# maniacs-ops/ringpop-go

Measured on AMD Instinct MI355X. Metric: simulated member-rounds/sec at 64k members, higher is better.
Workload: dtype u32; 1 GPU; config3_cascade: 65536 members, 655 killed at r=10; rounds 5-592 timed (steady state, kill, suspect wave; faulty wave from r>=35 in window); members=65536, live_member_rounds=38153303, parallelism=1 GPU

## Files before the change

include/swimsim.h:

```cpp
#ifndef SWIMSIM_H
#define SWIMSIM_H
#include <stddef.h>
#include <stdint.h>

#ifdef __cplusplus
extern "C" {
#endif

#define SWIMSIM_ABI_VERSION 13

enum {
    SWIMSIM_OK = 0,
    SWIMSIM_EINVAL = -1,
    SWIMSIM_ENOMEM = -2,
    SWIMSIM_EHIP = -3,
    SWIMSIM_ECAPACITY = -4,
    SWIMSIM_ERANGE = -5
};

enum { SWIMSIM_ALIVE = 0, SWIMSIM_SUSPECT = 1, SWIMSIM_FAULTY = 2, SWIMSIM_LEAVE = 3, SWIMSIM_TOMBSTONE = 4,
       SWIMSIM_UNKNOWN = 7 };
#define SWIMSIM_SOURCE_NONE (-1)

typedef struct swimsim_config {
// ... 14 lines not shown
    uint64_t message_pool_bytes;
    uint32_t observer_begin, observer_end;
    const struct swimsim_tuning *tuning;
} swimsim_config;

typedef struct swimsim_tuning {
    int32_t hot_slots;
    int32_t dense_slots;
    int32_t cs_async;
    int32_t cs_async_rows;
    int32_t cs_narrow_rows;
    int32_t cs_ref;
    int32_t fault_inject;
    int32_t defer_test;
    int32_t cs_defer;
} swimsim_tuning;

enum {
    SWIMSIM_EV_KILL = 1,
    SWIMSIM_EV_REVIVE = 2,
    SWIMSIM_EV_REINCARNATE = 3,
    SWIMSIM_EV_LEAVE = 4,
    SWIMSIM_EV_PARTITION = 5,
    SWIMSIM_EV_HEAL = 6,
    SWIMSIM_EV_REAP = 7,
    SWIMSIM_EV_CLOCK = 8
};
typedef struct swimsim_event { uint32_t round; uint32_t kind; int32_t a; int32_t b; } swimsim_event;

enum {
// ... 127 lines not shown
```

ringpop-go_amd/csrc/swimsim_device.h:

```cpp
#pragma once
#include <hip/hip_runtime.h>
#include <stdint.h>

namespace swimdev {

constexpr uint32_t ST_ALIVE = 0, ST_SUSPECT = 1, ST_FAULTY = 2, ST_LEAVE = 3, ST_TOMB = 4, ST_UNKNOWN = 7;
constexpr uint32_t SRC_NONE = 0xFFFFFFFFu;
constexpr uint32_t NO_DEADLINE = 0xFFFFFFFFu;
constexpr uint8_t DP_NONE = 0xFF;
constexpr uint32_t DE_NONE = 0xFFFFFFFFu;
__host__ __device__ inline uint32_t de_p(uint32_t x) { return x >> 24; }
__host__ __device__ inline uint32_t de_src(uint32_t x) { return (x & 0xFFFFFFu) == 0xFFFFFFu ? SRC_NONE : (x & 0xFFFFFFu); }
__host__ __device__ inline uint32_t de_x(uint32_t src, uint32_t p) { return (src & 0xFFFFFFu) | (p << 24); }

enum Counter {
    C_ROUNDS, C_PINGS, C_PINGS_OK, C_PINGREQS, C_HELPER_CALLS, C_HELPER_ERRORS, C_INCONCLUSIVE,
    C_SUSPECT_DECL, C_APPLIED, C_REFUTES, C_FULL_SYNCS, C_FULL_SYNCS_PINGREQ, C_RFS_DONE, C_RFS_OMITTED,
    C_TIMERS_FIRED, C_MSG_CHANGES, C_HEAL_ATTEMPTS, C_HEAL_FAILURES, C_NCOUNTERS,
    C_X_MERGED = C_NCOUNTERS, C_X_APPLIED, C_X_ISSUED, C_X_CS_ROWS, C_X_CS_DUP,
    C_X_MERGED_R, C_X_APPLIED_R, C_X_RISSUED, C_X_RCALLS, C_X_BUMPED, C_X_CS_ROWS_N, C_X_CSD_SCANNED,
    C_X_DENSE_RESP, C_X_DENSE_JOBS, C_X_JOBS_APPLIED, C_X_DENSE_HEAL,
    C_X_DEFER, C_X_DEFER_EQ, C_X_DEFER_NOROW, C_X_DEFER_REP, C_X_DEFER_UNDO,
    C_X_DEFER_REP_DIFF, C_X_DEFER_UNDO_DIFF, C_X_DEFER_FS, C_X_DEFER_UNDO_OVER, C_X_DEFER_CLEAN,
    C_X_ISSUE_SNAPS, C_X_LAZY_LATE, C_X_LAZY_MAT, C_NALL
};

constexpr int CTR_SHARDS = 64, CTR_STRIDE = 64;
static_assert(C_NALL <= CTR_STRIDE, "counter block too small");
constexpr uint32_t POOL_SHARDS = 64, POOL_CUR_STRIDE = 16;

enum ErrBits : uint32_t {
    E_POOL = 1, E_DENSE = 2, E_ECAP = 4, E_SHORT = 8, E_ITER = 16, E_COUNT = 32, E_XCAP = 64
};

struct MsgDesc {
    uint32_t off_lo, off_hi;
    uint32_t len;
    uint32_t kind;
};
// ... 238 lines not shown
```

ringpop-go_amd/csrc/swimsim_engine.hip:

```cpp
#include "swimsim_kernels.hip"
#include "swimsim_xchg.hip"
#include "swimsim_census.hip"
#include "swimsim_route.hip"

#include <hipcub/hipcub.hpp>
#include <rccl/rccl.h>

#include <algorithm>
#include <cmath>
#include <condition_variable>
#include <cstdarg>
#include <cstdio>
#include <cstring>
#include <memory>
#include <mutex>
#include <string>
#include <thread>
#include <vector>

#include "../../include/swimsim.h"

using namespace swimdev;

namespace {
// ... 335 lines not shown
    size_t rt_bytes_cap = 0, rt_keys_cap = 0, rt_rows_cap = 0, rt_own_cap = 0, rt_exc_cap = 0, rt_cub_bytes = 0;
    std::vector<uint64_t> rt_rel;
    hipEvent_t rt_ev[2] = {nullptr, nullptr};
    int csr_mode = 1;
    CsrSet csr, csr2;
    size_t csr_sbw_words = 0;
    uint32_t csr_ecap = 4096, csr_rcap = 1024, csr_KP = 0;
    uint64_t csr_launches = 0;
    uint32_t csr_side_min = 4097;
    int fault_inject = 0;
    int defer_test = 0;
    int cs_defer = 1;
    uint32_t rounds_left = 0;
    uint32_t round_deferred = 0;
    bool cs_carried = false;
    bool cs_defer_log = false;
    uint64_t cs_skipped_rounds = 0, cs_carried_rows = 0, cs_forced = 0, cs_units_base[3] = {0, 0, 0};
    bool colx_stale = false;
    std::string err;

    int fail(int code, const char *fmt, ...) {
        char buf[512];
        va_list ap;
        va_start(ap, fmt);
        vsnprintf(buf, sizeof buf, fmt, ap);
        va_end(ap);
        err = buf;
        return code;
    }
};
// ... 685 lines not shown
    if (remote) {
        hipLaunchKernelGGL(k_x_csresp, dim3(blocks_for_threads(h->keycap)), dim3(256), 0, h->s, h->d, h->csreq,
                           h->csreqcnt, h->xitems, h->xcnt, h->xcap, sS);
        if (int rc = xchg(h)) return rc;
    }
    Scope sc(h, phase == 1 ? F_PINGREQ : F_RECVFIN);
    hipLaunchKernelGGL(k_recv_finish, dim3(blocks_for_threads(maxn)), dim3(256), 0, h->s, h->d, h->defer,
                       h->defer_cnt, rdesc, phase, h->fsflag, h->rcs, h->defer_eq, sS);
    return 0;
}

int run_waves(swimsim *h, int phase, uint32_t maxpairs) {
    RecvArgs a{};
    a.counts = h->counts; a.offs = h->offs; a.ulist = h->ulist;
    a.phase = phase;
    a.sdesc = phase == 0 ? h->sdesc : h->sdesc2;
    a.sI = phase == 0 ? h->sI : h->sI2;
    a.sC = phase == 0 ? h->sC : h->sC2;
    a.sS = phase == 0 ? h->sS : h->sS2;
    a.rdesc = phase == 0 ? h->rdesc : h->rdesc2;
    a.defer = h->defer;
    a.defer_cnt = h->defer_cnt;
    a.fsflag = h->fsflag;
    a.r = h->round;
    a.pinfo = h->pinfo;
    {
        Scope sc(h, F_SORT);
        hipLaunchKernelGGL(k_pair_info, dim3(blocks_for_threads(std::max(h->inbox_n, h->NL))), dim3(256), 0, h->s, h->d,
                           h->vals_in, h->run_of, h->counts, h->offs, h->inbox_n, phase, a.sdesc, a.sI, a.sC, a.sS,
                           h->pinfo, h->vals_out, h->defer_cnt);
// ... 529 lines not shown
        hipEventCreateWithFlags(&h->ev_rt, hipEventDisableTiming) != hipSuccess) {
        h->err = "hipStreamCreate / hipEventCreate failed";
        return bail(SWIMSIM_EHIP);
    }
    const swimsim_tuning *tun = cfg->tuning;
    if (tun && tun->cs_async >= 0) h->cs_async = tun->cs_async != 0;
    if (tun && tun->cs_narrow_rows >= 0) h->cs_narrow_rows = (uint32_t)tun->cs_narrow_rows;
    if (tun && tun->cs_ref >= 0) h->csr_mode = tun->cs_ref;
    if (tun && tun->fault_inject > 0) h->fault_inject = tun->fault_inject;
    if (tun && tun->defer_test > 0) h->defer_test = tun->defer_test;
    if (tun && tun->cs_defer >= 0) h->cs_defer = tun->cs_defer;
    if (const char *v = getenv("SWIMSIM_CS_DEFER")) h->cs_defer = atoi(v);
    if (const char *v = getenv("SWIMSIM_CS_DEFER_LOG")) h->cs_defer_log = atoi(v) != 0;
    if (h->cs_defer < 0 || h->cs_defer > 2) {
        h->err = "swimsim_tuning.cs_defer is -1, 0, 1 or 2";
        return bail(SWIMSIM_EINVAL);
    }
    if (h->fault_inject & 32) h->csr_ecap = 24;
    if (h->fault_inject & 256) h->csr_side_min = 1024;
    if (const char *v = getenv("SWIMSIM_SYNC_SPIN")) h->sync_spin = atoi(v) != 0;
    if (const char *v = getenv("SWIMSIM_SIDE2"))
        if (atoi(v) == 0 && h->side2) { hipStreamDestroy(h->side2); h->side2 = nullptr; }
    DS &d = h->d;
    d.N = h->N; d.NP = h->NP; d.NL = h->NL; d.lo = h->lo;
    d.NB = h->NP / 64;
    d.NBW = (d.NB + 63) / 64;
    d.NBIT = ((h->NP / 32) + 3) & ~3u;
    d.W = h->W; d.pfactor = h->pfactor; d.K = h->K; d.maxjobs = h->maxjobs;
    d.to_susp = h->to_susp; d.to_faulty = h->to_faulty; d.to_tomb = h->to_tomb;
    d.seed = h->seed;
// ... 1101 lines not shown

int swimsim_kernel_times(swimsim_t *h, const char **names, double *avg_ms, uint64_t *launches, double *alg_bytes,
                         size_t cap, size_t *n) {
    if (!h) return SWIMSIM_EINVAL;
    drain_timing(h);
    uint64_t c[CTR_STRIDE];
    if (int rc = read_counters(h, c)) return rc;
    const double merged = (double)(c[C_X_MERGED] - h->fam_bytes_base[C_X_MERGED]);
    const double applied = (double)(c[C_X_APPLIED] - h->fam_bytes_base[C_X_APPLIED]);
    const double issued = (double)(c[C_X_ISSUED] - h->fam_bytes_base[C_X_ISSUED]);
    const double csrows = (double)(c[C_X_CS_ROWS] - h->fam_bytes_base[C_X_CS_ROWS]);
    const double csdups = (double)(c[C_X_CS_DUP] - h->fam_bytes_base[C_X_CS_DUP]);
    auto delta = [&](int k) { return (double)(c[k] - h->fam_bytes_base[k]); };
    const double merge_bytes = merged * 22.0 + applied * 23.0;
    const double resp_bytes = delta(C_X_MERGED_R) * 22.0 + delta(C_X_APPLIED_R) * 23.0 + delta(C_X_BUMPED) * 24.0;
    const double recv_issue_bytes = delta(C_X_RISSUED) * 36.0 + delta(C_X_RCALLS) * 4.0 * h->d.NBIT;
    for (int f = 0; f < F_NFAM && (size_t)f < cap; f++) {
        if (names) names[f] = kFamName[f];
        if (avg_ms) avg_ms[f] = h->fam_n[f] ? h->fam_ms[f] / (double)h->fam_n[f] : 0.0;
        if (launches) launches[f] = h->fam_n[f];
        if (alg_bytes) {
            double b = 0;
            if (f == F_CS_WIDE) b = csrows * 5.0 * h->N;
            if (f == F_CS_NARROW) b = delta(C_X_CS_ROWS_N) * 5.0 * h->N;
            if (f == F_CSPREP) b = csdups * 8.0 * h->N;
            if (f == F_CSD_SCAN) b = delta(C_X_CSD_SCANNED) * 4.0 * h->N;
            if (f == F_ISSUE) b = issued * 32.0;
            if (f == F_RECV) b = merge_bytes + recv_issue_bytes;
            if (f == F_RESP) b = resp_bytes;
            if (f == F_JOBS_MERGE) b = delta(C_X_DENSE_JOBS) * 5.0 * h->N + delta(C_X_JOBS_APPLIED) * 23.0;
            alg_bytes[f] = b;
        }
    }
    if (n) *n = F_NFAM;
    return SWIMSIM_OK;
}

int swimsim_kernel_units(swimsim_t *h, const char **names, double *values, size_t cap, size_t *n) {
    if (!h) return SWIMSIM_EINVAL;
    uint64_t c[CTR_STRIDE];
    if (int rc = read_counters(h, c)) return rc;
    static const char *kn[] = {"cs_rows_wide", "cs_rows_narrow", "cs_dup_rows", "recv_merged", "recv_applied",
                               "recv_issued", "recv_calls", "resp_merged", "resp_applied", "resp_bumped", "issued",
                               "bitmap_words_per_row", "hot_slots", "dense_resp", "dense_jobs", "jobs_applied",
                               "dense_heal", "defer", "defer_eq", "defer_norow", "defer_rep", "defer_undo",
                               "defer_rep_diff", "defer_undo_diff", "defer_fs", "defer_undo_over", "defer_clean",
                               "issue_snaps", "lazy_late", "lazy_mat",
                               "cs_skipped_rounds", "cs_carried_rows", "cs_forced"};
    const int ki[] = {C_X_CS_ROWS, C_X_CS_ROWS_N, C_X_CS_DUP, C_X_MERGED, C_X_APPLIED, C_X_RISSUED, C_X_RCALLS,
                      C_X_MERGED_R, C_X_APPLIED_R, C_X_BUMPED, C_X_ISSUED, -1, -2, C_X_DENSE_RESP, C_X_DENSE_JOBS,
                      C_X_JOBS_APPLIED, C_X_DENSE_HEAL, C_X_DEFER, C_X_DEFER_EQ, C_X_DEFER_NOROW, C_X_DEFER_REP,
                      C_X_DEFER_UNDO, C_X_DEFER_REP_DIFF, C_X_DEFER_UNDO_DIFF, C_X_DEFER_FS, C_X_DEFER_UNDO_OVER,
                      C_X_DEFER_CLEAN, C_X_ISSUE_SNAPS, C_X_LAZY_LATE, C_X_LAZY_MAT,
                      -3, -4, -5};
    const uint64_t lazy_c[3] = {h->cs_skipped_rounds - h->cs_units_base[0], h->cs_carried_rows - h->cs_units_base[1],
                                h->cs_forced - h->cs_units_base[2]};
    static_assert(sizeof(kn) / sizeof(kn[0]) == sizeof(ki) / sizeof(ki[0]), "one counter per name");
    uint32_t hot = 0;
    if (h->d.hot_cnt) {
        HIPCHK(h, hipMemcpyAsync(&hot, h->d.hot_cnt, 4, hipMemcpyDeviceToHost, h->s));
        HIPCHK(h, stream_sync(h));
    }
    const size_t k = sizeof(ki) / sizeof(ki[0]);
    for (size_t i = 0; i < k && i < cap; i++) {
        if (names) names[i] = kn[i];
        if (values)
            values[i] = ki[i] == -1 ? (double)h->d.NBIT : ki[i] == -2 ? (double)hot : ki[i] <= -3 ? (double)lazy_c[-3 - ki[i]]
                                                                                : (double)(c[ki[i]] - h->fam_bytes_base[ki[i]]);
// ... 197 lines not shown
```

ringpop-go_amd/csrc/swimsim_kernels.hip:

```cpp
#include "swimsim_kernels.h"

namespace swimdev {

#define SWIM_DPP(old, src, ctrl, rm) ((uint32_t)__builtin_amdgcn_update_dpp((int)(old), (int)(src), (ctrl), (rm), 0xf, false))
template <typename Op>
__device__ __forceinline__ uint32_t dpp_scan(uint32_t x, uint32_t id, Op op) {
    x = op(x, SWIM_DPP(id, x, 0x111, 0xf));
    x = op(x, SWIM_DPP(id, x, 0x112, 0xf));
    x = op(x, SWIM_DPP(id, x, 0x114, 0xf));
    x = op(x, SWIM_DPP(id, x, 0x118, 0xf));
    x = op(x, SWIM_DPP(id, x, 0x142, 0xa));
    x = op(x, SWIM_DPP(id, x, 0x143, 0xc));
    return x;
}
__device__ __forceinline__ uint32_t dpp_scan_add(uint32_t x) { return dpp_scan(x, 0u, [](uint32_t a, uint32_t b) { return a + b; }); }
__device__ __forceinline__ uint32_t dpp_scan_umin(uint32_t x) {
    return dpp_scan(x, 0xFFFFFFFFu, [](uint32_t a, uint32_t b) { return min(a, b); });
}
__device__ __forceinline__ int32_t dpp_scan_imax(int32_t x) {
    return (int32_t)dpp_scan((uint32_t)x, 0x80000000u, [](uint32_t a, uint32_t b) { return (uint32_t)max((int32_t)a, (int32_t)b); });
}
__device__ __forceinline__ int32_t dpp_scan_imin(int32_t x) {
    return (int32_t)dpp_scan((uint32_t)x, 0x7FFFFFFFu, [](uint32_t a, uint32_t b) { return (uint32_t)min((int32_t)a, (int32_t)b); });
}
// ... 330 lines not shown
                merge_change_w(d, ol, o, m, cur[u], w[u] & 7u, w[u] >> 3, meta.x, meta.y, now_e, sched_r, acc);
        }
    }
}

__device__ __forceinline__ void merge_first(const DS &d, const MsgDesc &md, uint4 (&rec)[MB]) {
    const unsigned long long off = ((unsigned long long)md.off_hi << 32) | md.off_lo;
#pragma unroll
    for (int u = 0; u < MB; u++) {
        const uint32_t i = u * 64 + lane_id();
        rec[u] = md.kind == 0 && i < md.len ? d.pool[off + i] : make_uint4(0xFFFFFFFFu, 0, 0, 0);
    }
}
__device__ __forceinline__ void wave_merge_body(const DS &d, uint32_t ol, uint32_t o, const MsgDesc &md, uint32_t now_e,
                                                uint32_t sched_r, MAcc &acc, int dctr, const uint4 *pre0 = nullptr,
                                                uint32_t *ulog = nullptr, LazyCtx *lz = nullptr) {
    const uint32_t *rowp = d.mw + (size_t)ol * d.NP;
    const uint32_t *hrow = d.hmw + (size_t)ol * d.HP;
    if (md.kind == 0) {
        const unsigned long long off = ((unsigned long long)md.off_hi << 32) | md.off_lo;
        for (uint32_t base = 0; base < md.len; base += 64 * MB) {
            uint4 rec[MB];
            uint32_t cur[MB], hk[MB];
#pragma unroll
            for (int u = 0; u < MB; u++) {
                const uint32_t i = base + u * 64 + lane_id();
                rec[u] = pre0 && base == 0 ? pre0[u] : i < md.len ? d.pool[off + i] : make_uint4(0xFFFFFFFFu, 0, 0, 0);
            }
#pragma unroll
            for (int u = 0; u < MB; u++) hk[u] = rec[u].x != 0xFFFFFFFFu ? rec_slot(d, rec[u]) : SRC_NONE;
#pragma unroll
            for (int u = 0; u < MB; u++)
                cur[u] = rec[u].x == 0xFFFFFFFFu ? 0u : hk[u] != SRC_NONE ? hrow[hk[u]] : rowp[rec_m(rec[u])];
#pragma unroll
            for (int u = 0; u < MB; u++) {
                const int before = acc.napp;
                if (rec[u].x != 0xFFFFFFFFu)
                    merge_change_w(d, ol, o, rec_m(rec[u]), cur[u], rec_st(rec[u]), rec_e(rec[u]), rec[u].z, rec[u].w, now_e,
                                   sched_r, acc, hk[u]);
                if (ulog) {
                    const bool ap = acc.napp != before;
                    const unsigned long long b = __ballot(ap);
                    const uint32_t at = *ulog + (uint32_t)__popcll(b & lanemask_lt());
                    if (ap && at < d.ulog_stride) d.ulog[(size_t)ol * d.ulog_stride + at] = make_uint2(rec_m(rec[u]), cur[u]);
                    *ulog += (uint32_t)__popcll(b);
                }
            }
            if (ulog && lz && lz->pend && *ulog > d.ulog_cap) wave_lazy_late(d, ol, o, *lz, *ulog);
        }
    } else if (md.kind == 1) {
        if (ulog && lz && lz->pend) wave_lazy_late(d, ol, o, *lz, *ulog);
        wave_merge_dense(d, ol, o, md, now_e, sched_r, acc);
        if (dctr >= 0 && lane_id() == 0) ctr_add(d, dctr, 1ull);
        if (ulog) *ulog = d.ulog_cap + 1u;
    }
    __threadfence_block();
}
__device__ void wave_merge_msg(const DS &d, uint32_t ol, uint32_t o, const MsgDesc &md, uint32_t now_e, uint32_t sched_r,
                               int cset = 0, int dctr = -1) {
    MAcc acc;
    acc_begin(d, ol, acc);
    wave_merge_body(d, ol, o, md, now_e, sched_r, acc, dctr);
    wave_finalize(d, ol, acc, cset);
}
__device__ __forceinline__ void wave_merge_msg_pre(const DS &d, uint32_t ol, uint32_t o, const MsgDesc &md, uint32_t now_e,
                                                   uint32_t sched_r, int cset, RowPre &p, int dctr = -1,
                                                   const uint4 *pre0 = nullptr, bool logit = false,
                                                   LazyCtx *lz = nullptr) {
    MAcc acc;
    acc.tag = p.useq;
    wave_merge_body(d, ol, o, md, now_e, sched_r, acc, dctr, pre0, logit && d.ulog ? &p.ulog : nullptr, lz);
    wave_finalize_pre(d, ol, acc, cset, p);
}

__device__ __forceinline__ int2 wave_bump_body(const DS &d, uint32_t ol, const MsgDesc &md, int maxp) {
    if (md.kind != 0) return make_int2(0, 0);
    const unsigned long long off = ((unsigned long long)md.off_hi << 32) | md.off_lo;
    uint32_t *dx = (uint32_t *)(d.dent + (size_t)ol * d.NP);
    uint32_t *hx = (uint32_t *)(d.hde + (size_t)ol * d.HP);
    int del = 0, delnh = 0;
    for (uint32_t base = 0; base < md.len; base += 64 * MB) {
        uint32_t m[MB], x[MB], hk[MB];
#pragma unroll
        for (int u = 0; u < MB; u++) {
            const uint32_t i = base + u * 64 + lane_id();
            const uint2 xy = i < md.len ? *(const uint2 *)(d.pool + off + i) : make_uint2(0xFFFFFFFFu, 0u);
// ... 61 lines not shown
__device__ __forceinline__ unsigned long long pool_alloc(const DS &d, uint32_t n) {
    unsigned long long off = 0;
    if (lane_id() == 0 && n) off = pool_alloc_lane0(d, n);
    return bcast64(off);
}

__device__ __forceinline__ uint32_t wscan_excl(uint32_t v, uint32_t &total) {
    const uint32_t x = dpp_scan_add(v);
    total = lane63(x);
    return x - v;
}

template <bool RECV>
__device__ __forceinline__ uint32_t wave_issue_body(const DS &d, uint32_t ol, uint32_t sender, uint32_t sinc, MsgDesc &out,
                                                    uint32_t cnt, int maxp, bool hotwalk, uint32_t nslots,
                                                    unsigned long long off, int &del_out, int &delnh_out) {
    const size_t rb = (size_t)ol * d.NP, hb = (size_t)ol * d.HP;
    uint32_t *bits = d.dbit + (size_t)ol * d.NBIT;
    uint32_t pos = 0;
    int del = 0, delnh = 0;
    if (hotwalk) {
        for (uint32_t base = 0; base < nslots; base += 64 * MB) {
            uint2 ce[MB];
            uint32_t wv[MB], m[MB];
#pragma unroll
            for (int u = 0; u < MB; u++) {
                const uint32_t k = base + u * 64 + lane_id();
                ce[u] = k < nslots ? d.hde[hb + k] : make_uint2(DE_NONE, 0);
                wv[u] = k < nslots ? d.hmw[hb + k] : 0u;
                m[u] = k < nslots ? d.hlist[k] : 0u;
            }
            bool keep[MB];
            uint32_t nk = 0;
#pragma unroll
            for (int u = 0; u < MB; u++) {
                const uint32_t src = de_src(ce[u].x);
                keep[u] = de_p(ce[u].x) != DP_NONE && !(RECV && src == sender && ce[u].y == sinc);
                nk += keep[u] ? 1u : 0u;
            }
            uint32_t tot;
            uint32_t at = pos + wscan_excl(nk, tot);
#pragma unroll
            for (int u = 0; u < MB; u++) {
                if (!keep[u]) continue;
                const uint32_t st = (wv[u] & 7u) == ST_UNKNOWN ? ST_TOMB : (wv[u] & 7u);
                if (at < cnt) d.pool[off + at] = rec_make(m[u], st, wv[u] >> 3, de_src(ce[u].x), ce[u].y, base + u * 64 + lane_id() + 1u);
                at++;
                if (RECV) {
                    const uint32_t k = base + u * 64 + lane_id();
                    uint32_t nx;
                    if ((int)(de_p(ce[u].x) + 1) >= maxp) {
                        nx = ce[u].x | 0xFF000000u;
                        atomicAnd(bits + (m[u] >> 5), ~(1u << (m[u] & 31)));
                        del++;
                    } else {
                        nx = ce[u].x + (1u << 24);
                    }
                    d.hde[hb + k].x = nx;
                }
            }
            pos += tot;
        }
    } else if ((uint64_t)cnt * 4u > d.NP) {
        const uint2 *dcell = d.dent + rb;
        const uint32_t *drow = d.mw + rb;
        for (uint32_t base = 0; base < d.NP; base += 64 * MB) {
            uint2 ce[MB];
            uint32_t wv[MB], hk[MB];
#pragma unroll
            for (int u = 0; u < MB; u++) {
                const uint32_t m = base + u * 64 + lane_id();
                const bool in = m < d.N;
                hk[u] = in && d.hidx ? d.hidx[m] : SRC_NONE;
                ce[u] = in ? dcell[m] : make_uint2(DE_NONE, 0);
                wv[u] = in ? drow[m] : 0u;
            }
#pragma unroll
            for (int u = 0; u < MB; u++)
                if (hk[u] != SRC_NONE) {
                    ce[u] = d.hde[hb + hk[u]];
                    wv[u] = d.hmw[hb + hk[u]];
                }
            bool keep[MB];
            uint32_t nk = 0;
#pragma unroll
            for (int u = 0; u < MB; u++) {
                keep[u] = de_p(ce[u].x) != DP_NONE &&
                          !(RECV && de_src(ce[u].x) == sender && ce[u].y == sinc);
                nk += keep[u] ? 1u : 0u;
            }
            uint32_t tot;
            uint32_t at = pos + wscan_excl(nk, tot);
#pragma unroll
            for (int u = 0; u < MB; u++) {
                const uint32_t m = base + u * 64 + lane_id();
                bool gone = false;
                if (keep[u]) {
                    const uint32_t st = (wv[u] & 7u) == ST_UNKNOWN ? ST_TOMB : (wv[u] & 7u);
                    if (at < cnt) d.pool[off + at] = rec_make(m, st, wv[u] >> 3, de_src(ce[u].x), ce[u].y, tag_of_slot(hk[u]));
                    at++;
                    if (RECV) {
                        uint32_t nx;
                        if ((int)(de_p(ce[u].x) + 1) >= maxp) {
                            nx = ce[u].x | 0xFF000000u;
                            gone = true;
                            del++;
                            delnh += hk[u] == SRC_NONE;
                        } else {
                            nx = ce[u].x + (1u << 24);
                        }
                        if (hk[u] != SRC_NONE) d.hde[hb + hk[u]].x = nx;
                        else d.dent[rb + m].x = nx;
                    }
                }
                if (RECV) {
// ... 19 lines not shown
            const uint32_t w3 = __hip_atomic_load(bp + 3, __ATOMIC_RELAXED, __HIP_MEMORY_SCOPE_AGENT);
            lo = ((unsigned long long)w1 << 32) | w0;
            hi = ((unsigned long long)w3 << 32) | w2;
        }
        const uint32_t mbase = q * 32;
        unsigned long long dlo = 0, dhi = 0;
        while (__any(lo != 0 || hi != 0)) {
            uint32_t m[MB];
#pragma unroll
            for (int k = 0; k < MB; k++) {
                if (lo) { m[k] = mbase + (uint32_t)(__ffsll((long long)lo) - 1); lo &= lo - 1; }
                else if (hi) { m[k] = mbase + 64 + (uint32_t)(__ffsll((long long)hi) - 1); hi &= hi - 1; }
                else m[k] = 0xFFFFFFFFu;
            }
            uint2 ce[MB];
            uint32_t wv[MB], hk[MB];
#pragma unroll
            for (int k = 0; k < MB; k++) hk[k] = m[k] != 0xFFFFFFFFu ? hot_slot(d, m[k]) : SRC_NONE;
#pragma unroll
            for (int k = 0; k < MB; k++) {
                if (m[k] == 0xFFFFFFFFu) {
                    ce[k] = make_uint2(DE_NONE, 0);
                    wv[k] = 0u;
                } else if (hk[k] != SRC_NONE) {
                    ce[k] = d.hde[hb + hk[k]];
                    wv[k] = d.hmw[hb + hk[k]];
                } else {
                    ce[k] = d.dent[rb + m[k]];
                    wv[k] = d.mw[rb + m[k]];
                }
            }
            uint32_t p[MB];
            uint2 sr[MB];
#pragma unroll
            for (int k = 0; k < MB; k++) {
                p[k] = de_p(ce[k].x);
                sr[k] = make_uint2(de_src(ce[k].x), ce[k].y);
            }
            bool keep[MB];
            uint32_t nk = 0;
#pragma unroll
            for (int k = 0; k < MB; k++) {
                keep[k] = m[k] != 0xFFFFFFFFu && !(RECV && sr[k].x == sender && sr[k].y == sinc);
                nk += keep[k] ? 1u : 0u;
            }
            uint32_t tot;
            uint32_t at = pos + wscan_excl(nk, tot);
#pragma unroll
            for (int k = 0; k < MB; k++) {
                if (!keep[k]) continue;
                const uint32_t st = (wv[k] & 7u) == ST_UNKNOWN ? ST_TOMB : (wv[k] & 7u);
                if (at < cnt) d.pool[off + at] = rec_make(m[k], st, wv[k] >> 3, sr[k].x, sr[k].y, tag_of_slot(hk[k]));
                at++;
                if (RECV) {
                    uint32_t nx;
                    if ((int)(p[k] + 1) >= maxp) {
                        nx = ce[k].x | 0xFF000000u;
                        const uint32_t l = m[k] - mbase;
                        if (l < 64) dlo |= 1ull << l; else dhi |= 1ull << (l - 64);
                        del++;
                        delnh += hk[k] == SRC_NONE;
                    } else {
                        nx = ce[k].x + (1u << 24);
                    }
                    if (hk[k] != SRC_NONE) d.hde[hb + hk[k]].x = nx;
                    else d.dent[rb + m[k]].x = nx;
                }
            }
// ... 3 lines not shown
            if (dlo & 0xFFFFFFFFull) atomicAnd(bits + q + 0, ~(uint32_t)dlo);
            if (dlo >> 32) atomicAnd(bits + q + 1, ~(uint32_t)(dlo >> 32));
            if (dhi & 0xFFFFFFFFull) atomicAnd(bits + q + 2, ~(uint32_t)dhi);
            if (dhi >> 32) atomicAnd(bits + q + 3, ~(uint32_t)(dhi >> 32));
        }
    }
    if (RECV) {
        del_out = wsum(del);
        delnh_out = wsum(delnh);
    } else if (pos != cnt && lane_id() == 0) {
        atomicOr(d.err, E_COUNT);
    }
    out.off_lo = (uint32_t)off;
    out.off_hi = (uint32_t)(off >> 32);
    out.len = min(pos, cnt);
    return out.len;
}

template <bool RECV>
__device__ uint32_t wave_issue_t(const DS &d, uint32_t ol, uint32_t sender, uint32_t sinc, MsgDesc &out) {
    const uint32_t cnt = (uint32_t)d.dcnt[ol];
    const int maxp = RECV ? d.maxp[ol] : 0;
    const bool hotwalk = d.hidx && d.nhe[ol] == 0;
    const uint32_t nslots = d.hidx ? d.hot_cnt[0] : 0u;
    out.kind = 0; out.len = 0; out.off_lo = out.off_hi = 0;
    if (cnt == 0) return 0;
    const unsigned long long off = pool_alloc(d, cnt);
    if (off == ~0ull) return 0;
    int del = 0, delnh = 0;
    const uint32_t n = wave_issue_body<RECV>(d, ol, sender, sinc, out, cnt, maxp, hotwalk, nslots, off, del, delnh);
    if (RECV) {
// ... 608 lines not shown
    const unsigned long long k = keys[i];
    const uint32_t u = (uint32_t)(k >> 32) - d.lo;
    if (u >= d.NL) return;
    const uint32_t p = offs[u] + kslot[i];
    vals_in[p] = (uint32_t)k;
    run_of[p] = u;
}

struct RecvArgs {
    const uint32_t *counts, *offs;
    const uint32_t *ulist;
    const uint4 *pinfo;
    int phase;
    const MsgDesc *sdesc;
    const uint32_t *sI, *sC;
    uint32_t *sS;
    MsgDesc *rdesc;
    uint4 *defer;
    uint32_t *defer_cnt;
    uint8_t *fsflag;
    uint32_t r;
};

constexpr uint32_t RANK_LANE_MAX = 64;
__global__ void k_pair_info(const DS d, const uint32_t *vals_in, const uint32_t *run_of, const uint32_t *counts,
                            const uint32_t *offs, uint32_t n, int phase, const MsgDesc *sdesc, const uint32_t *sI,
                            const uint32_t *sC, const uint32_t *sS, uint4 *pinfo, uint32_t *vals_out, uint32_t *defer_cnt) {
    const uint32_t i = blockIdx.x * blockDim.x + threadIdx.x;
    if (d.ulog_cnt && i < d.NL) d.ulog_cnt[i] = 0u;
    if (i == 0) *defer_cnt = 0u;
// ... 18 lines not shown
            for (int k = 0; k < 64; k++) rk += (uint32_t)__builtin_amdgcn_readlane((int)x, k) < v;
        }
        if (mine) rank = rk;
        todo &= ~__ballot(mine);
    }
    if (!valid) return;
    const uint32_t p = off + rank, sender = phase == 0 ? v : v / d.K;
    vals_out[p] = v;
    if (sender >= d.N) return;
    const MsgDesc md = sdesc[sender];
    pinfo[2 * (size_t)p] = make_uint4(md.off_lo, md.off_hi, md.len, md.kind);
    pinfo[2 * (size_t)p + 1] = make_uint4(sI[sender], sC[sender], sS ? sS[sender] : SRC_NONE, v);
}

__device__ __forceinline__ void recv_one_pre(const DS &d, const RecvArgs &a, uint32_t j, const uint4 pi0, const uint4 pi1,
                                             uint32_t pair, uint32_t nslots, uint32_t now, RowPre &p, LazyCtx &lz) {
    const uint32_t ol = j - d.lo;
    const uint32_t v = pi1.w, sender = a.phase == 0 ? v : v / d.K, resp_idx = v;
    MsgDesc md;
    md.off_lo = pi0.x; md.off_hi = pi0.y; md.len = pi0.z; md.kind = pi0.w;
    const uint64_t bound = (uint64_t)(uint32_t)p.dcnt + md.len;
    const bool early = md.kind == 0 && bound > 0 && bound <= min(4096ull, d.pool_cap / POOL_SHARDS / 16);
    unsigned long long roff = 0;
    if (early && lane_id() == 0) roff = pool_alloc_lane0(d, (uint32_t)bound);
    wave_merge_msg_pre(d, ol, j, md, now, now, 0, p, -1, nullptr, true, &lz);
    MsgDesc resp;
    resp.kind = 0; resp.len = 0; resp.off_lo = resp.off_hi = 0;
    uint32_t kept = 0;
    const uint32_t cnt = (uint32_t)p.dcnt;
    if (cnt) {
        const unsigned long long off = early ? bcast64(roff) : pool_alloc(d, cnt);
        if (off != ~0ull) {
            int del = 0, delnh = 0;
            kept = wave_issue_body<true>(d, ol, sender, pi1.x, resp, cnt, p.maxp, d.hidx && p.nhe == 0, nslots, off, del,
                                         delnh);
            if (del) { p.dcnt -= del; if (lane_id() == 0) d.dcnt[ol] = p.dcnt; }
            if (delnh) { p.nhe -= delnh; if (lane_id() == 0) d.nhe[ol] = p.nhe; }
            __threadfence_block();
        }
    }
    if (lane_id() == 0) {
        ctr_add(d, C_X_RISSUED, (unsigned long long)kept);
        ctr_add(d, C_X_RCALLS, 1ull);
    }
    if (kept == 0) {
        const uint32_t scs = pi1.y;
        const uint32_t sslot = a.sS ? pi1.z : SRC_NONE;
        const bool rdirty = p.dirty != 0;
        const uint32_t rpend = rdirty ? SRC_NONE : p.cpslot;
        if (rdirty || rpend != SRC_NONE || sslot != SRC_NONE) {
            if (wave_snapshot(d, ol, j, resp) && lane_id() == 0) {
                if (rpend != SRC_NONE) d.dense_meta[resp.off_lo].w = rpend + 1u;
                else if (!rdirty) d.dense_cs[resp.off_lo] = p.cs;
                a.defer[atomicAdd(a.defer_cnt, 1u)] =
                    make_uint4(resp_idx | (rdirty ? 0x80000000u : 0u), resp.off_lo, sslot != SRC_NONE ? sslot : scs,
                               pair | (sslot != SRC_NONE ? 0x80000000u : 0u));
            }
            resp.kind = 2;
        } else if (p.cs != scs) {
            wave_snapshot(d, ol, j, resp);
            if (lane_id() == 0) {
                if (a.phase == 0) a.fsflag[pair] = 1;
                ctr_add(d, a.phase == 0 ? C_FULL_SYNCS : C_FULL_SYNCS_PINGREQ, 1ull);
            }
        }
    }
    if (lane_id() == 0) {
        a.rdesc[resp_idx] = resp;
        if (resp.kind != 2) ctr_add(d, C_MSG_CHANGES, (unsigned long long)resp.len);
        if (a.phase == 1) {
            ctr_add(d, C_HELPER_CALLS, 1ull);
            ctr_add(d, C_MSG_CHANGES, (unsigned long long)md.len);
        }
    }
}

constexpr int RECV_MIN_WAVES = 4;
__global__ void __launch_bounds__(256, RECV_MIN_WAVES) k_recv(DS d, RecvArgs a) {
    const uint32_t w = wave_gid();
    if (w >= d.NL) return;
    const uint32_t u = a.ulist[w];
    if (w >= a.offs[d.NL + 1]) return;
    const uint32_t n = a.counts[u], off = a.offs[u], key = d.lo + u;
    RowPre p = row_pre(d, key - d.lo);
    const uint32_t now = wave_clock(d, key, a.r);
    const uint32_t nslots = d.hidx ? d.hot_cnt[0] : 0u;
    LazyCtx lz;
    lz.sS = a.sS; lz.sI = a.sI;
    lz.pend = a.sS && d.ulog && uni(a.sS[key]) == SRC_PEND;
    for (uint32_t w = 0; w < n; w++) {
        const uint32_t pair = off + w;
        recv_one_pre(d, a, key, a.pinfo[2 * (size_t)pair], a.pinfo[2 * (size_t)pair + 1], pair, nslots, now, p, lz);
    }
    if (d.ulog_cnt && lane_id() == 0) d.ulog_cnt[key - d.lo] = min(p.ulog, d.ulog_cap + 1u);
}

__global__ void k_colx_rebuild(DS d) {
    const uint32_t m = blockIdx.x * blockDim.x + threadIdx.x;
    bool diff = false;
    if (m < d.N) {
        const uint32_t w0 = d.mw[m];
        for (uint32_t ol = 1; ol < d.NL && !diff; ol++) diff = d.mw[(size_t)ol * d.NP + m] != w0;
    }
    const unsigned long long bits = __ballot(diff);
    const uint32_t w = (m & ~63u) >> 5;
    if (lane_id() == 0) {
        if (w < d.NBIT) d.colx[w] = (uint32_t)bits;
// ... 294 lines not shown
    }
}

__global__ void k_resp(DS d, const int32_t *tgt, const uint8_t *failed, const MsgDesc *sdesc, const MsgDesc *rdesc,
                       uint32_t r) {
    const uint32_t ol = wave_gid();
    if (ol >= d.NL) return;
    if (tgt[ol] < 0 || failed[ol]) return;
    const uint32_t o = d.lo + ol;
    RowPre p = row_pre(d, ol);
    const uint32_t now = wave_clock(d, o, r);
    const MsgDesc sd = sdesc[o], rd = rdesc[o];
    uint4 rec0[MB];
    merge_first(d, rd, rec0);
    wave_bump_pre(d, ol, sd, p);
    wave_merge_msg_pre(d, ol, o, rd, now, now, 1, p, C_X_DENSE_RESP, rec0);
    if (lane_id() == 0) {
        ctr_add(d, C_PINGS_OK, 1ull);
        if (sd.kind == 0) ctr_add(d, C_X_BUMPED, (unsigned long long)sd.len);
    }
}

__global__ void k_resolve(DS d, const int32_t *tgt, const uint8_t *failed, const uint32_t *H, const uint32_t *nh,
                          const MsgDesc *sdesc2, const MsgDesc *rdesc2, uint32_t r) {
    const uint32_t ol = wave_gid();
    if (ol >= d.NL || !failed[ol]) return;
    const uint32_t o = d.lo + ol, K = d.K;
    const uint32_t now = wave_clock(d, o, r);
    uint32_t errs = 0;
    for (uint32_t q = 0; q < nh[ol]; q++) {
        const uint32_t h = H[(size_t)ol * K + q];
        if (!reach(d, o, h)) {
            errs++;
            wave_bump(d, ol, sdesc2[o]);
        } else {
            wave_merge_msg(d, ol, o, rdesc2[(size_t)o * K + q], now, now, 2, C_X_DENSE_RESP);
        }
    }
    if (lane_id() == 0) {
        if (errs) ctr_add(d, C_HELPER_ERRORS, (unsigned long long)errs);
        if (errs == K) {
            ctr_add(d, C_INCONCLUSIVE, 1ull);
        } else {
            ctr_add(d, C_SUSPECT_DECL, 1ull);
            const uint32_t t = (uint32_t)tgt[ol];
            const uint32_t te = d.mw[(size_t)ol * d.NP + t] >> 3;
            thread_make_change(d, ol, o, t, te, ST_SUSPECT, now);
        }
    }
}

// ... 370 lines not shown
```

ringpop-go_amd/swimsim/__init__.py:

```python
from __future__ import annotations

import ctypes as C
import os
from dataclasses import dataclass

import numpy as np

_HERE = os.path.dirname(os.path.abspath(__file__))
LIB_PATH = os.path.join(_HERE, "libswimsim.so")

ALIVE, SUSPECT, FAULTY, LEAVE, TOMBSTONE, UNKNOWN = 0, 1, 2, 3, 4, 7
STATUS_NAMES = {ALIVE: "alive", SUSPECT: "suspect", FAULTY: "faulty", LEAVE: "leave", TOMBSTONE: "tombstone"}
SOURCE_NONE = -1
EV_KILL, EV_REVIVE, EV_REINCARNATE, EV_LEAVE, EV_PARTITION, EV_HEAL, EV_REAP = 1, 2, 3, 4, 5, 6, 7
EV_CLOCK = 8
COUNTER_NAMES = [
    "rounds", "pings", "pings_ok", "pingreqs", "helper_calls", "helper_errors", "inconclusive",
    "suspect_decl", "applied", "refutes", "full_syncs", "full_syncs_pingreq", "rfs_done",
    "rfs_omitted", "timers_fired", "msg_changes", "heal_attempts", "heal_failures",
]
T0_MS = 1_500_000_000_000
CENSUS_LIVE, CENSUS_ALL = 0, 1
CENSUS_WHO = {"live": CENSUS_LIVE, "all": CENSUS_ALL}
ROUTE_N_REPLICAS = 16
# ... 8 lines not shown
class Config(C.Structure):
    _fields_ = [
        ("num_members", C.c_uint32), ("device", C.c_uint32), ("t0_ms", C.c_int64),
        ("protocol_period_ms", C.c_uint32), ("suspect_timeout_ms", C.c_uint32), ("faulty_timeout_ms", C.c_uint32),
        ("tombstone_timeout_ms", C.c_uint32), ("ping_request_size", C.c_uint32),
        ("max_reverse_full_sync_jobs", C.c_uint32), ("p_factor", C.c_uint32), ("seed", C.c_uint64),
        ("addresses", C.c_char_p), ("addr_stride", C.c_uint32), ("max_rounds", C.c_uint32),
        ("message_pool_bytes", C.c_uint64), ("observer_begin", C.c_uint32), ("observer_end", C.c_uint32),
        ("tuning", C.c_void_p),
    ]


class Tuning(C.Structure):
    _fields_ = [("hot_slots", C.c_int32), ("dense_slots", C.c_int32), ("cs_async", C.c_int32),
                ("cs_async_rows", C.c_int32), ("cs_narrow_rows", C.c_int32), ("cs_ref", C.c_int32),
                ("fault_inject", C.c_int32), ("defer_test", C.c_int32), ("cs_defer", C.c_int32)]


def make_tuning(tuning):
    if not tuning:
        return None
    t = Tuning(*([-1] * len(Tuning._fields_)))
    for k, v in tuning.items():
        if k not in dict(Tuning._fields_):
            raise ValueError(f"unknown tuning field {k}")
        setattr(t, k, int(v))
    return t


class Event(C.Structure):
    _fields_ = [("round", C.c_uint32), ("kind", C.c_uint32), ("a", C.c_int32), ("b", C.c_int32)]
# ... 1030 lines not shown
```

Baseline: 118.4 million member-rounds/s.

## Elide echoing sender's just-merged changes from ping responses via shared bitmap

During receive merge, each wave records in a per-wave shared-memory bitmap the hot-slot changes whose merged state already matches what the sender sent. When it builds the response, it skips writing those records to the message pool, so they are not sent back to the sender. Merging an empty response is now skipped entirely. The aim is to cut pool writes and response-merge work in steady state. The cost is extra shared memory per block, which may reduce occupancy, plus atomics and bitmap clearing per message. It also relies on the echoed records being redundant for correctness.

```diff
diff --git a/include/swimsim.h b/include/swimsim.h
--- a/include/swimsim.h
+++ b/include/swimsim.h
@@ -7,7 +7,7 @@
 extern "C" {
 #endif
 
-#define SWIMSIM_ABI_VERSION 13
+#define SWIMSIM_ABI_VERSION 14
 
 enum {
     SWIMSIM_OK = 0,
@@ -52,6 +52,7 @@
     int32_t fault_inject;
     int32_t defer_test;
     int32_t cs_defer;
+    int32_t resp_echo;
 } swimsim_tuning;
 
 enum {
diff --git a/ringpop-go_amd/csrc/swimsim_device.h b/ringpop-go_amd/csrc/swimsim_device.h
--- a/ringpop-go_amd/csrc/swimsim_device.h
+++ b/ringpop-go_amd/csrc/swimsim_device.h
@@ -22,7 +22,8 @@
     C_X_DENSE_RESP, C_X_DENSE_JOBS, C_X_JOBS_APPLIED, C_X_DENSE_HEAL,
     C_X_DEFER, C_X_DEFER_EQ, C_X_DEFER_NOROW, C_X_DEFER_REP, C_X_DEFER_UNDO,
     C_X_DEFER_REP_DIFF, C_X_DEFER_UNDO_DIFF, C_X_DEFER_FS, C_X_DEFER_UNDO_OVER, C_X_DEFER_CLEAN,
-    C_X_ISSUE_SNAPS, C_X_LAZY_LATE, C_X_LAZY_MAT, C_NALL
+    C_X_ISSUE_SNAPS, C_X_LAZY_LATE, C_X_LAZY_MAT,
+    C_X_ECHO, C_NALL
 };
 
 constexpr int CTR_SHARDS = 64, CTR_STRIDE = 64;
diff --git a/ringpop-go_amd/csrc/swimsim_engine.hip b/ringpop-go_amd/csrc/swimsim_engine.hip
--- a/ringpop-go_amd/csrc/swimsim_engine.hip
+++ b/ringpop-go_amd/csrc/swimsim_engine.hip
@@ -373,6 +373,7 @@
     uint32_t rounds_left = 0;
     uint32_t round_deferred = 0;
     bool cs_carried = false;
+    int resp_echo = 1;
     bool cs_defer_log = false;
     uint64_t cs_skipped_rounds = 0, cs_carried_rows = 0, cs_forced = 0, cs_units_base[3] = {0, 0, 0};
     bool colx_stale = false;
@@ -1088,6 +1089,7 @@
     RecvArgs a{};
     a.counts = h->counts; a.offs = h->offs; a.ulist = h->ulist;
     a.phase = phase;
+    a.echo = h->resp_echo;
     a.sdesc = phase == 0 ? h->sdesc : h->sdesc2;
     a.sI = phase == 0 ? h->sI : h->sI2;
     a.sC = phase == 0 ? h->sC : h->sC2;
@@ -1647,6 +1649,12 @@
     if (const char *v = getenv("SWIMSIM_CS_DEFER_LOG")) h->cs_defer_log = atoi(v) != 0;
     if (h->cs_defer < 0 || h->cs_defer > 2) {
         h->err = "swimsim_tuning.cs_defer is -1, 0, 1 or 2";
+        return bail(SWIMSIM_EINVAL);
+    }
+    if (tun && tun->resp_echo >= 0) h->resp_echo = tun->resp_echo;
+    if (const char *v = getenv("SWIMSIM_RESP_ECHO")) h->resp_echo = atoi(v);
+    if (h->resp_echo < 0 || h->resp_echo > 1) {
+        h->err = "swimsim_tuning.resp_echo is -1, 0 or 1";
         return bail(SWIMSIM_EINVAL);
     }
     if (h->fault_inject & 32) h->csr_ecap = 24;
@@ -2778,7 +2786,7 @@
     auto delta = [&](int k) { return (double)(c[k] - h->fam_bytes_base[k]); };
     const double merge_bytes = merged * 22.0 + applied * 23.0;
     const double resp_bytes = delta(C_X_MERGED_R) * 22.0 + delta(C_X_APPLIED_R) * 23.0 + delta(C_X_BUMPED) * 24.0;
-    const double recv_issue_bytes = delta(C_X_RISSUED) * 36.0 + delta(C_X_RCALLS) * 4.0 * h->d.NBIT;
+    const double recv_issue_bytes = delta(C_X_RISSUED) * 36.0 - delta(C_X_ECHO) * 16.0 + delta(C_X_RCALLS) * 4.0 * h->d.NBIT;
     for (int f = 0; f < F_NFAM && (size_t)f < cap; f++) {
         if (names) names[f] = kFamName[f];
         if (avg_ms) avg_ms[f] = h->fam_n[f] ? h->fam_ms[f] / (double)h->fam_n[f] : 0.0;
@@ -2809,13 +2817,13 @@
                                "bitmap_words_per_row", "hot_slots", "dense_resp", "dense_jobs", "jobs_applied",
                                "dense_heal", "defer", "defer_eq", "defer_norow", "defer_rep", "defer_undo",
                                "defer_rep_diff", "defer_undo_diff", "defer_fs", "defer_undo_over", "defer_clean",
-                               "issue_snaps", "lazy_late", "lazy_mat",
+                               "issue_snaps", "lazy_late", "lazy_mat", "resp_echoed",
                                "cs_skipped_rounds", "cs_carried_rows", "cs_forced"};
     const int ki[] = {C_X_CS_ROWS, C_X_CS_ROWS_N, C_X_CS_DUP, C_X_MERGED, C_X_APPLIED, C_X_RISSUED, C_X_RCALLS,
                       C_X_MERGED_R, C_X_APPLIED_R, C_X_BUMPED, C_X_ISSUED, -1, -2, C_X_DENSE_RESP, C_X_DENSE_JOBS,
                       C_X_JOBS_APPLIED, C_X_DENSE_HEAL, C_X_DEFER, C_X_DEFER_EQ, C_X_DEFER_NOROW, C_X_DEFER_REP,
                       C_X_DEFER_UNDO, C_X_DEFER_REP_DIFF, C_X_DEFER_UNDO_DIFF, C_X_DEFER_FS, C_X_DEFER_UNDO_OVER,
-                      C_X_DEFER_CLEAN, C_X_ISSUE_SNAPS, C_X_LAZY_LATE, C_X_LAZY_MAT,
+                      C_X_DEFER_CLEAN, C_X_ISSUE_SNAPS, C_X_LAZY_LATE, C_X_LAZY_MAT, C_X_ECHO,
                       -3, -4, -5};
     const uint64_t lazy_c[3] = {h->cs_skipped_rounds - h->cs_units_base[0], h->cs_carried_rows - h->cs_units_base[1],
                                 h->cs_forced - h->cs_units_base[2]};
diff --git a/ringpop-go_amd/csrc/swimsim_kernels.hip b/ringpop-go_amd/csrc/swimsim_kernels.hip
--- a/ringpop-go_amd/csrc/swimsim_kernels.hip
+++ b/ringpop-go_amd/csrc/swimsim_kernels.hip
@@ -368,7 +368,8 @@
 }
 __device__ __forceinline__ void wave_merge_body(const DS &d, uint32_t ol, uint32_t o, const MsgDesc &md, uint32_t now_e,
                                                 uint32_t sched_r, MAcc &acc, int dctr, const uint4 *pre0 = nullptr,
-                                                uint32_t *ulog = nullptr, LazyCtx *lz = nullptr) {
+                                                uint32_t *ulog = nullptr, LazyCtx *lz = nullptr, uint32_t *echo = nullptr,
+                                                uint32_t echo_sender = 0) {
     const uint32_t *rowp = d.mw + (size_t)ol * d.NP;
     const uint32_t *hrow = d.hmw + (size_t)ol * d.HP;
     if (md.kind == 0) {
@@ -388,10 +389,16 @@
                 cur[u] = rec[u].x == 0xFFFFFFFFu ? 0u : hk[u] != SRC_NONE ? hrow[hk[u]] : rowp[rec_m(rec[u])];
 #pragma unroll
             for (int u = 0; u < MB; u++) {
-                const int before = acc.napp;
+                const int before = acc.napp, refuted = acc.nref;
                 if (rec[u].x != 0xFFFFFFFFu)
                     merge_change_w(d, ol, o, rec_m(rec[u]), cur[u], rec_st(rec[u]), rec_e(rec[u]), rec[u].z, rec[u].w, now_e,
                                    sched_r, acc, hk[u]);
+                if (echo && hk[u] != SRC_NONE) {
+                    const uint32_t recw = (rec_e(rec[u]) << 3) | rec_st(rec[u]);
+                    const bool same = acc.napp != before ? acc.nref == refuted : cur[u] == recw;
+                    if (same && rec_st(rec[u]) != ST_TOMB && rec_m(rec[u]) != echo_sender)
+                        atomicOr(echo + (hk[u] >> 5), 1u << (hk[u] & 31));
+                }
                 if (ulog) {
                     const bool ap = acc.napp != before;
                     const unsigned long long b = __ballot(ap);
@@ -408,6 +415,7 @@
         if (dctr >= 0 && lane_id() == 0) ctr_add(d, dctr, 1ull);
         if (ulog) *ulog = d.ulog_cap + 1u;
     }
+    if (echo) __builtin_amdgcn_fence(__ATOMIC_RELEASE, "wavefront");
     __threadfence_block();
 }
 __device__ void wave_merge_msg(const DS &d, uint32_t ol, uint32_t o, const MsgDesc &md, uint32_t now_e, uint32_t sched_r,
@@ -420,10 +428,12 @@
 __device__ __forceinline__ void wave_merge_msg_pre(const DS &d, uint32_t ol, uint32_t o, const MsgDesc &md, uint32_t now_e,
                                                    uint32_t sched_r, int cset, RowPre &p, int dctr = -1,
                                                    const uint4 *pre0 = nullptr, bool logit = false,
-                                                   LazyCtx *lz = nullptr) {
+                                                   LazyCtx *lz = nullptr, uint32_t *echo = nullptr,
+                                                   uint32_t echo_sender = 0) {
     MAcc acc;
     acc.tag = p.useq;
-    wave_merge_body(d, ol, o, md, now_e, sched_r, acc, dctr, pre0, logit && d.ulog ? &p.ulog : nullptr, lz);
+    wave_merge_body(d, ol, o, md, now_e, sched_r, acc, dctr, pre0, logit && d.ulog ? &p.ulog : nullptr, lz, echo,
+                    echo_sender);
     wave_finalize_pre(d, ol, acc, cset, p);
 }
 
@@ -515,29 +525,36 @@
 template <bool RECV>
 __device__ __forceinline__ uint32_t wave_issue_body(const DS &d, uint32_t ol, uint32_t sender, uint32_t sinc, MsgDesc &out,
                                                     uint32_t cnt, int maxp, bool hotwalk, uint32_t nslots,
-                                                    unsigned long long off, int &del_out, int &delnh_out) {
+                                                    unsigned long long off, int &del_out, int &delnh_out,
+                                                    const uint32_t *echo = nullptr) {
     const size_t rb = (size_t)ol * d.NP, hb = (size_t)ol * d.HP;
     uint32_t *bits = d.dbit + (size_t)ol * d.NBIT;
     uint32_t pos = 0;
+    uint32_t kept = 0;
     int del = 0, delnh = 0;
+    const bool skip = RECV && echo != nullptr;
+    auto echo_word = [&](uint32_t hk) { return skip && hk != SRC_NONE ? echo[hk >> 5] : 0u; };
     if (hotwalk) {
         for (uint32_t base = 0; base < nslots; base += 64 * MB) {
             uint2 ce[MB];
-            uint32_t wv[MB], m[MB];
+            uint32_t wv[MB], m[MB], ew[MB];
 #pragma unroll
             for (int u = 0; u < MB; u++) {
                 const uint32_t k = base + u * 64 + lane_id();
                 ce[u] = k < nslots ? d.hde[hb + k] : make_uint2(DE_NONE, 0);
                 wv[u] = k < nslots ? d.hmw[hb + k] : 0u;
                 m[u] = k < nslots ? d.hlist[k] : 0u;
-            }
-            bool keep[MB];
+                ew[u] = echo_word(k < nslots ? k : SRC_NONE);
+            }
+            bool keep[MB], wr[MB];
             uint32_t nk = 0;
 #pragma unroll
             for (int u = 0; u < MB; u++) {
                 const uint32_t src = de_src(ce[u].x);
                 keep[u] = de_p(ce[u].x) != DP_NONE && !(RECV && src == sender && ce[u].y == sinc);
-                nk += keep[u] ? 1u : 0u;
+                wr[u] = keep[u] && !((ew[u] >> (lane_id() & 31)) & 1u);
+                kept += keep[u] ? 1u : 0u;
+                nk += wr[u] ? 1u : 0u;
             }
             uint32_t tot;
             uint32_t at = pos + wscan_excl(nk, tot);
@@ -545,8 +562,10 @@
             for (int u = 0; u < MB; u++) {
                 if (!keep[u]) continue;
                 const uint32_t st = (wv[u] & 7u) == ST_UNKNOWN ? ST_TOMB : (wv[u] & 7u);
-                if (at < cnt) d.pool[off + at] = rec_make(m[u], st, wv[u] >> 3, de_src(ce[u].x), ce[u].y, base + u * 64 + lane_id() + 1u);
-                at++;
+                if (wr[u]) {
+                    if (at < cnt) d.pool[off + at] = rec_make(m[u], st, wv[u] >> 3, de_src(ce[u].x), ce[u].y, base + u * 64 + lane_id() + 1u);
+                    at++;
+                }
                 if (RECV) {
                     const uint32_t k = base + u * 64 + lane_id();
                     uint32_t nx;
@@ -567,7 +586,7 @@
         const uint32_t *drow = d.mw + rb;
         for (uint32_t base = 0; base < d.NP; base += 64 * MB) {
             uint2 ce[MB];
-            uint32_t wv[MB], hk[MB];
+            uint32_t wv[MB], hk[MB], ew[MB];
 #pragma unroll
             for (int u = 0; u < MB; u++) {
                 const uint32_t m = base + u * 64 + lane_id();
@@ -577,18 +596,22 @@
                 wv[u] = in ? drow[m] : 0u;
             }
 #pragma unroll
-            for (int u = 0; u < MB; u++)
+            for (int u = 0; u < MB; u++) {
+                ew[u] = echo_word(hk[u]);
                 if (hk[u] != SRC_NONE) {
                     ce[u] = d.hde[hb + hk[u]];
                     wv[u] = d.hmw[hb + hk[u]];
                 }
-            bool keep[MB];
+            }
+            bool keep[MB], wr[MB];
             uint32_t nk = 0;
 #pragma unroll
             for (int u = 0; u < MB; u++) {
                 keep[u] = de_p(ce[u].x) != DP_NONE &&
                           !(RECV && de_src(ce[u].x) == sender && ce[u].y == sinc);
-                nk += keep[u] ? 1u : 0u;
+                wr[u] = keep[u] && !((ew[u] >> (hk[u] & 31)) & 1u);
+                kept += keep[u] ? 1u : 0u;
+                nk += wr[u] ? 1u : 0u;
             }
             uint32_t tot;
             uint32_t at = pos + wscan_excl(nk, tot);
@@ -598,8 +621,10 @@
                 bool gone = false;
                 if (keep[u]) {
                     const uint32_t st = (wv[u] & 7u) == ST_UNKNOWN ? ST_TOMB : (wv[u] & 7u);
-                    if (at < cnt) d.pool[off + at] = rec_make(m, st, wv[u] >> 3, de_src(ce[u].x), ce[u].y, tag_of_slot(hk[u]));
-                    at++;
+                    if (wr[u]) {
+                        if (at < cnt) d.pool[off + at] = rec_make(m, st, wv[u] >> 3, de_src(ce[u].x), ce[u].y, tag_of_slot(hk[u]));
+                        at++;
+                    }
                     if (RECV) {
                         uint32_t nx;
                         if ((int)(de_p(ce[u].x) + 1) >= maxp) {
@@ -649,11 +674,12 @@
                 else m[k] = 0xFFFFFFFFu;
             }
             uint2 ce[MB];
-            uint32_t wv[MB], hk[MB];
+            uint32_t wv[MB], hk[MB], ew[MB];
 #pragma unroll
             for (int k = 0; k < MB; k++) hk[k] = m[k] != 0xFFFFFFFFu ? hot_slot(d, m[k]) : SRC_NONE;
 #pragma unroll
             for (int k = 0; k < MB; k++) {
+                ew[k] = echo_word(hk[k]);
                 if (m[k] == 0xFFFFFFFFu) {
                     ce[k] = make_uint2(DE_NONE, 0);
                     wv[k] = 0u;
@@ -672,12 +698,14 @@
                 p[k] = de_p(ce[k].x);
                 sr[k] = make_uint2(de_src(ce[k].x), ce[k].y);
             }
-            bool keep[MB];
+            bool keep[MB], wr[MB];
             uint32_t nk = 0;
 #pragma unroll
             for (int k = 0; k < MB; k++) {
                 keep[k] = m[k] != 0xFFFFFFFFu && !(RECV && sr[k].x == sender && sr[k].y == sinc);
-                nk += keep[k] ? 1u : 0u;
+                wr[k] = keep[k] && !((ew[k] >> (hk[k] & 31)) & 1u);
+                kept += keep[k] ? 1u : 0u;
+                nk += wr[k] ? 1u : 0u;
             }
             uint32_t tot;
             uint32_t at = pos + wscan_excl(nk, tot);
@@ -685,8 +713,10 @@
             for (int k = 0; k < MB; k++) {
                 if (!keep[k]) continue;
                 const uint32_t st = (wv[k] & 7u) == ST_UNKNOWN ? ST_TOMB : (wv[k] & 7u);
-                if (at < cnt) d.pool[off + at] = rec_make(m[k], st, wv[k] >> 3, sr[k].x, sr[k].y, tag_of_slot(hk[k]));
-                at++;
+                if (wr[k]) {
+                    if (at < cnt) d.pool[off + at] = rec_make(m[k], st, wv[k] >> 3, sr[k].x, sr[k].y, tag_of_slot(hk[k]));
+                    at++;
+                }
                 if (RECV) {
                     uint32_t nx;
                     if ((int)(p[k] + 1) >= maxp) {
@@ -720,7 +750,7 @@
     out.off_lo = (uint32_t)off;
     out.off_hi = (uint32_t)(off >> 32);
     out.len = min(pos, cnt);
-    return out.len;
+    return skip ? min((uint32_t)wsum((int)kept), cnt) : out.len;
 }
 
 template <bool RECV>
@@ -1359,6 +1389,7 @@
     int phase;
     const MsgDesc *sdesc;
     const uint32_t *sI, *sC;
+    int echo;
     uint32_t *sS;
     MsgDesc *rdesc;
     uint4 *defer;
@@ -1407,16 +1438,20 @@
 }
 
 __device__ __forceinline__ void recv_one_pre(const DS &d, const RecvArgs &a, uint32_t j, const uint4 pi0, const uint4 pi1,
-                                             uint32_t pair, uint32_t nslots, uint32_t now, RowPre &p, LazyCtx &lz) {
+                                             uint32_t pair, uint32_t nslots, uint32_t now, RowPre &p, LazyCtx &lz,
+                                             uint32_t *echo) {
     const uint32_t ol = j - d.lo;
     const uint32_t v = pi1.w, sender = a.phase == 0 ? v : v / d.K, resp_idx = v;
     MsgDesc md;
     md.off_lo = pi0.x; md.off_hi = pi0.y; md.len = pi0.z; md.kind = pi0.w;
+    if (md.kind != 0) echo = nullptr;
+    if (echo)
+        for (uint32_t i = lane_id(); i < (nslots + 31u) / 32u; i += 64) echo[i] = 0u;
     const uint64_t bound = (uint64_t)(uint32_t)p.dcnt + md.len;
     const bool early = md.kind == 0 && bound > 0 && bound <= min(4096ull, d.pool_cap / POOL_SHARDS / 16);
     unsigned long long roff = 0;
     if (early && lane_id() == 0) roff = pool_alloc_lane0(d, (uint32_t)bound);
-    wave_merge_msg_pre(d, ol, j, md, now, now, 0, p, -1, nullptr, true, &lz);
+    wave_merge_msg_pre(d, ol, j, md, now, now, 0, p, -1, nullptr, true, &lz, echo, sender);
     MsgDesc resp;
     resp.kind = 0; resp.len = 0; resp.off_lo = resp.off_hi = 0;
     uint32_t kept = 0;
@@ -1426,7 +1461,7 @@
         if (off != ~0ull) {
             int del = 0, delnh = 0;
             kept = wave_issue_body<true>(d, ol, sender, pi1.x, resp, cnt, p.maxp, d.hidx && p.nhe == 0, nslots, off, del,
-                                         delnh);
+                                         delnh, echo);
             if (del) { p.dcnt -= del; if (lane_id() == 0) d.dcnt[ol] = p.dcnt; }
             if (delnh) { p.nhe -= delnh; if (lane_id() == 0) d.nhe[ol] = p.nhe; }
             __threadfence_block();
@@ -1435,6 +1470,7 @@
     if (lane_id() == 0) {
         ctr_add(d, C_X_RISSUED, (unsigned long long)kept);
         ctr_add(d, C_X_RCALLS, 1ull);
+        if (a.phase == 0 && kept != resp.len) ctr_add(d, C_X_ECHO, (unsigned long long)(kept - resp.len));
     }
     if (kept == 0) {
         const uint32_t scs = pi1.y;
@@ -1460,7 +1496,7 @@
     }
     if (lane_id() == 0) {
         a.rdesc[resp_idx] = resp;
-        if (resp.kind != 2) ctr_add(d, C_MSG_CHANGES, (unsigned long long)resp.len);
+        if (resp.kind != 2) ctr_add(d, C_MSG_CHANGES, (unsigned long long)(resp.kind == 0 ? kept : resp.len));
         if (a.phase == 1) {
             ctr_add(d, C_HELPER_CALLS, 1ull);
             ctr_add(d, C_MSG_CHANGES, (unsigned long long)md.len);
@@ -1469,7 +1505,10 @@
 }
 
 constexpr int RECV_MIN_WAVES = 4;
+constexpr uint32_t ECHO_WORDS = (RT_MAXSLOTS + 31u) / 32u + 2u;
+static_assert(ECHO_WORDS * 32u >= RT_COLD, "a record's slot tag indexes the echo bitmap");
 __global__ void __launch_bounds__(256, RECV_MIN_WAVES) k_recv(DS d, RecvArgs a) {
+    __shared__ uint32_t echo_bits[4][ECHO_WORDS];
     const uint32_t w = wave_gid();
     if (w >= d.NL) return;
     const uint32_t u = a.ulist[w];
@@ -1481,9 +1520,10 @@
     LazyCtx lz;
     lz.sS = a.sS; lz.sI = a.sI;
     lz.pend = a.sS && d.ulog && uni(a.sS[key]) == SRC_PEND;
+    uint32_t *echo = a.echo && d.hidx ? echo_bits[(threadIdx.x >> 6) & 3u] : nullptr;
     for (uint32_t w = 0; w < n; w++) {
         const uint32_t pair = off + w;
-        recv_one_pre(d, a, key, a.pinfo[2 * (size_t)pair], a.pinfo[2 * (size_t)pair + 1], pair, nslots, now, p, lz);
+        recv_one_pre(d, a, key, a.pinfo[2 * (size_t)pair], a.pinfo[2 * (size_t)pair + 1], pair, nslots, now, p, lz, echo);
     }
     if (d.ulog_cnt && lane_id() == 0) d.ulog_cnt[key - d.lo] = min(p.ulog, d.ulog_cap + 1u);
 }
@@ -1808,7 +1848,8 @@
     uint4 rec0[MB];
     merge_first(d, rd, rec0);
     wave_bump_pre(d, ol, sd, p);
-    wave_merge_msg_pre(d, ol, o, rd, now, now, 1, p, C_X_DENSE_RESP, rec0);
+    if (rd.kind != 0 || rd.len)
+        wave_merge_msg_pre(d, ol, o, rd, now, now, 1, p, C_X_DENSE_RESP, rec0);
     if (lane_id() == 0) {
         ctr_add(d, C_PINGS_OK, 1ull);
         if (sd.kind == 0) ctr_add(d, C_X_BUMPED, (unsigned long long)sd.len);
@@ -1828,7 +1869,8 @@
             errs++;
             wave_bump(d, ol, sdesc2[o]);
         } else {
-            wave_merge_msg(d, ol, o, rdesc2[(size_t)o * K + q], now, now, 2, C_X_DENSE_RESP);
+            const MsgDesc rd = rdesc2[(size_t)o * K + q];
+            if (rd.kind != 0 || rd.len) wave_merge_msg(d, ol, o, rd, now, now, 2, C_X_DENSE_RESP);
         }
     }
     if (lane_id() == 0) {
diff --git a/ringpop-go_amd/swimsim/__init__.py b/ringpop-go_amd/swimsim/__init__.py
--- a/ringpop-go_amd/swimsim/__init__.py
+++ b/ringpop-go_amd/swimsim/__init__.py
@@ -46,7 +46,8 @@
 class Tuning(C.Structure):
     _fields_ = [("hot_slots", C.c_int32), ("dense_slots", C.c_int32), ("cs_async", C.c_int32),
                 ("cs_async_rows", C.c_int32), ("cs_narrow_rows", C.c_int32), ("cs_ref", C.c_int32),
-                ("fault_inject", C.c_int32), ("defer_test", C.c_int32), ("cs_defer", C.c_int32)]
+                ("fault_inject", C.c_int32), ("defer_test", C.c_int32), ("cs_defer", C.c_int32),
+                ("resp_echo", C.c_int32)]
 
 
 def make_tuning(tuning):
```

Result: faster. 126.0 million member-rounds/s (median of 6 runs) (+6.4%).
